# Gadersd/stable-diffusion-burn

Hardware: AMD Instinct MI355X
Metric: images/sec @512x512, 20-step DDIM CFG=7.5, SD v1.4 (higher is better)
Workload: dtype f32

## Files before the change

### ffi/sdmi.rs

```rust
use std::error::Error;
use std::ffi::{c_char, c_double, c_float, c_int, c_void, CStr, CString};

#[repr(C)]
pub struct SdmiConfig {
    pub device: i32,
    pub model_channels: i32,
    pub n_head: i32,
    pub ctx_dim: i32,
    pub latent_h: i32,
    pub latent_w: i32,
    pub vae_ch: i32,
    pub max_batch: i32,
    pub precision: i32,
    pub clip_layers: i32,
    pub clip_heads: i32,
    pub clip_vocab: i32,
    pub clip_ctx: i32,
    pub unet_in_ch: i32,
    pub reserved: [i32; 2],
}

impl SdmiConfig {
    pub fn control_hint_ch(&self) -> i32 { self.reserved[0] }
    pub fn set_control_hint_ch(&mut self, v: i32) { self.reserved[0] = v; }
    pub fn variant(&self) -> i32 { self.reserved[1] }
    pub fn set_variant(&mut self, v: i32) { self.reserved[1] = v; }
}

#[repr(C)]
#[derive(Default, Debug, Clone, Copy)]
pub struct SdmiAttnPlan {
    pub kernel: i32,
    pub waves: i32,
    pub q_rows: i32,
    pub kv_tile: i32,
    pub kv_splits: i32,
    pub reserved: [i32; 3],
}

#[repr(C)]
pub struct SdmiControl {
    pub hint_rgb: *const u8,
    pub n_hint: i32,
    pub hint_h: i32,
    pub hint_w: i32,
    pub strength: f64,
    pub start: f64,
    pub end: f64,
    pub reserved: [i64; 4],
}

#[repr(C)]
pub struct SdmiSampler {
    pub kind: i32,
    pub reserved0: i32,
    pub eta: f64,
    pub noise_seed: u64,
    pub image_base: i64,
    pub reserved: [i64; 4],
}
// ... 764 lines not shown
```

### include/sdmi.h

```cpp
#ifndef SDMI_H
#define SDMI_H

#include <stddef.h>
#include <stdint.h>

#ifdef __cplusplus
extern "C" {
#endif

typedef struct sdmi_ctx sdmi_ctx;

typedef enum sdmi_status {
    SDMI_OK = 0,
    SDMI_ERR_INVALID = -1,
    SDMI_ERR_HIP = -2,
    SDMI_ERR_WEIGHTS = -3,
    SDMI_ERR_IO = -4,
    SDMI_ERR_UNSUPPORTED = -5,
    SDMI_ERR_STATE = -6
} sdmi_status;

typedef struct sdmi_config {
    int32_t device;
    int32_t model_channels;
// ... 288 lines not shown
                   float* out);
int sdmi_op_unpack_tensor(sdmi_ctx* ctx, const void* raw, int32_t dtype, int32_t ndim, const int64_t* dims, int32_t transform, float* out);
int sdmi_op_geglu_forward(sdmi_ctx* ctx, const float* x, const float* weight, const float* bias, int32_t rows, int32_t cin,
                          int32_t hidden, float* out);
int sdmi_op_timestep_embedding(sdmi_ctx* ctx, int32_t t, int32_t dim, float* out);
int sdmi_op_timestep_embedding_f(sdmi_ctx* ctx, double t, int32_t dim, float* out);

int sdmi_set_option(sdmi_ctx* ctx, const char* key, const char* value);
int sdmi_last_call_stats(sdmi_ctx* ctx, double* gpu_ms, int64_t* n_kernels, double* flops);
int sdmi_profile_stats(sdmi_ctx* ctx, int32_t cls, double* ms, int64_t* launches, double* flops, double* bytes);
int sdmi_profile_overhead(sdmi_ctx* ctx, double* ms);
int sdmi_bench_conv(sdmi_ctx* ctx, int32_t n, int32_t cin, int32_t h, int32_t w, int32_t cout,
                    int32_t k, int32_t stride, int32_t upsample2x, int32_t tile_cfg, int32_t splitk,
                    int32_t iters, double* ms_out);

int sdmi_bench_attention(sdmi_ctx* ctx, int32_t n, int32_t nq, int32_t nk, int32_t n_state, int32_t n_head,
                         int32_t iters, double* ms_out);
typedef struct sdmi_attn_plan {
    int32_t kernel;
    int32_t waves;
    int32_t q_rows;
    int32_t kv_tile;
    int32_t kv_splits;
    int32_t reserved[3];
} sdmi_attn_plan;
int sdmi_attention_plan(sdmi_ctx* ctx, int32_t n, int32_t n_head, int32_t nq, int32_t nk, int32_t d_head, int32_t has_mask, sdmi_attn_plan* out);

#ifdef __cplusplus
}
#endif
#endif
```

### stable_diffusion_burn_amd/_capi.py

```python
from __future__ import annotations

import ctypes as C
import os
import sys
from pathlib import Path

_PKG = Path(__file__).resolve().parent
LIB_PATH = _PKG / "lib" / "libsdmi.so"


class SdmiError(RuntimeError):
    def __init__(self, status: int, message: str):
        super().__init__(f"sdmi status {status}: {message}")
        self.status = status


class SdmiConfig(C.Structure):
    _fields_ = [
        ("device", C.c_int32), ("model_channels", C.c_int32), ("n_head", C.c_int32), ("ctx_dim", C.c_int32),
        ("latent_h", C.c_int32), ("latent_w", C.c_int32), ("vae_ch", C.c_int32), ("max_batch", C.c_int32),
        ("precision", C.c_int32), ("clip_layers", C.c_int32), ("clip_heads", C.c_int32), ("clip_vocab", C.c_int32),
        ("clip_ctx", C.c_int32), ("unet_in_ch", C.c_int32), ("reserved", C.c_int32 * 2),
    ]

    @property
    def control_hint_ch(self) -> int:
        return int(self.reserved[0])

    @control_hint_ch.setter
    def control_hint_ch(self, v: int) -> None:
        self.reserved[0] = int(v)

    @property
    def variant(self) -> int:
        return int(self.reserved[1])

    @variant.setter
    def variant(self, v: int) -> None:
        self.reserved[1] = int(v)


class SdmiAttnPlan(C.Structure):
    _fields_ = [("kernel", C.c_int32), ("waves", C.c_int32), ("q_rows", C.c_int32), ("kv_tile", C.c_int32), ("kv_splits", C.c_int32), ("reserved", C.c_int32 * 3)]


class SdmiOpView(C.Structure):
    _fields_ = [("in_ld", C.c_int32), ("in_off", C.c_int32), ("out_ld", C.c_int32), ("out_off", C.c_int32), ("in_fill", C.c_float),
                ("in_planes", C.c_int32), ("out_planes", C.c_int32)]


class SdmiSampler(C.Structure):
    _fields_ = [("kind", C.c_int32), ("reserved0", C.c_int32), ("eta", C.c_double), ("noise_seed", C.c_uint64), ("image_base", C.c_int64),
                ("reserved", C.c_int64 * 4)]


class SdmiKSampler(C.Structure):
    _fields_ = [("kind", C.c_int32), ("schedule", C.c_int32), ("eta", C.c_double), ("rho", C.c_double), ("sigma_min", C.c_double), ("sigma_max", C.c_double),
                ("noise_seed", C.c_uint64), ("image_base", C.c_int64), ("reserved", C.c_int64 * 4)]


class SdmiControl(C.Structure):
    _fields_ = [("hint_rgb", C.POINTER(C.c_uint8)), ("n_hint", C.c_int32), ("hint_h", C.c_int32), ("hint_w", C.c_int32), ("strength", C.c_double),
                ("start", C.c_double), ("end", C.c_double), ("reserved", C.c_int64 * 4)]


class SdmiInpaint(C.Structure):
# ... 188 lines not shown
```

### stable_diffusion_burn_amd/csrc/attn_plan.cpp

```cpp
#include "attn_plan.hpp"

#include <algorithm>

#include "error.hpp"

namespace sdmi {

static const int kCUs = 256;

static long long workgroups(const AttnPlanIn& p, int rows) { return (long long)((p.nq + rows - 1) / rows) * p.n * p.n_head; }

static AttnPlan form(const AttnPlanIn& p, AttnKernel k, int waves, int kv_splits = 1, int wpe = 1, int qr = 1) {
    const AttnGeom& g = *attn_geom(k, p.d_head, qr);
    AttnPlan a{};
    a.kernel = k; a.waves = waves; a.wpe = wpe; a.qr = qr;
    a.q_rows = g.rows_per_wave * waves; a.kv_tile = g.kv_tile; a.kv_splits = kv_splits;
    return a;
}

static int plan_kv_splits(const AttnPlanIn& p, const AttnPlanOpts& o, bool on_split) {
    if (p.bf16 || p.has_mask || o.attn_kv_splits == 1) return 1;
    const AttnGeom& g = *attn_geom(on_split ? AttnKernel::Split : AttnKernel::Flash, p.d_head);
    const int tiles = (p.nk + g.kv_tile - 1) / g.kv_tile;
    if (o.attn_kv_splits > 1) return std::min(o.attn_kv_splits, std::max(1, tiles));
    const long long most = std::min(tiles / 2, 8);
    const long long wgs4 = workgroups(p, 4 * g.rows_per_wave);
    long long s = std::min<long long>(wgs4 > 0 && wgs4 <= kCUs / 2 ? kCUs / wgs4 : 1, most);
    if (on_split && o.attn_kv_prefer8) {
        const long long wgs8 = workgroups(p, 8 * g.rows_per_wave);
        const long long s8 = std::min<long long>(wgs8 < kCUs ? (kCUs + wgs8 - 1) / wgs8 : 1, most);
        if (s8 >= 2 && wgs8 * s8 >= kCUs) s = s8;
    }
    return (int)std::max<long long>(1, s);
}

static bool d64_stays_on_flash(const AttnPlanIn& p, const AttnPlanOpts& o) {
    if (p.nq <= 64) return false;
    const int tiles = (p.nk + 63) / 64;
    const int sf = plan_kv_splits(p, o, false), ss = plan_kv_splits(p, o, true);
    if (workgroups(p, 64) * sf > kCUs) return false;
    const int tf = (tiles + sf - 1) / sf, ts = (tiles + ss - 1) / ss;
    return 8 * tf + (sf > 1 ? 15 : 0) <= 9 * ts + (ss > 1 ? 15 : 0);
}

static AttnPlan plan_flash(const AttnPlanIn& p, int kv_splits) {
    return form(p, AttnKernel::Flash, 2 * workgroups(p, 128) >= 3 * kCUs ? 8 : 4, kv_splits);
}

static AttnPlan plan_split(const AttnPlanIn& p, const AttnPlanOpts& o, int kv_splits) {
    const bool pk = p.d_head == 40 && (o.attn_pack_tail & 1), lg = (o.attn_pack_tail & 2) != 0;
    const bool w8 = workgroups(p, 256) * kv_splits >= kCUs && (lg || p.d_head != 80);
    AttnPlan a = form(p, AttnKernel::Split, w8 ? 8 : 4, kv_splits);
    a.pk = pk; a.lg = lg;
    return a;
}

static AttnPlan plan_bf16(const AttnPlanIn& p, const AttnPlanOpts& o) {
    const int v = o.attn_bf16_variant, d = p.d_head;
    const bool force = (v & 0x100) != 0, short_ctx = p.nk <= 128;
    auto fills = [&](int rows, int per_cu) { return workgroups(p, rows) >= per_cu * kCUs; };
    if (d == 40) {
        if ((v & 4) && (force ? !(v & 2) : short_ctx && fills(256, 2))) return form(p, AttnKernel::Bf16, 4, 1, 2, 2);
        if ((v & 2) && (force || (!short_ctx && fills(512, 1)))) return form(p, AttnKernel::Bf16, 8, 1, 2, 2);
    }
    if ((d == 40 || d == 80) && (v & 1) && (force || (short_ctx && fills(128, 2)))) return form(p, AttnKernel::Bf16, 4, 1, 2);
    for (int waves : {8, 4})
        if (fills(32 * waves, 1)) return form(p, AttnKernel::Bf16, waves);
    return form(p, AttnKernel::Bf16, 2);
}

AttnPlan plan_attention(const AttnPlanIn& p, const AttnPlanOpts& o) {
    const int d = p.d_head;
    const bool fused = attn_supported_head_dim(d);
    if (p.planes_out && (p.bf16 || !fused || (p.n_head * d) % 32)) throw Error(SDMI_ERR_STATE, "attention: plane output needs a fused fp32 kernel");
    if (!fused) {
        if (p.has_mask) throw Error(SDMI_ERR_UNSUPPORTED, "attention: additive mask is only supported for head dims 40/80/160");
        if (d % 32) throw Error(SDMI_ERR_UNSUPPORTED, "attention: head dim must be 40/80/160 or a multiple of 32");
        if (p.bf16 && (d % 64)) throw Error(SDMI_ERR_UNSUPPORTED, "bf16 attention (unfused path): head dim must be a multiple of 64");
        AttnPlan a{};
        a.kernel = AttnKernel::Unfused; a.kv_splits = 1;
        return a;
    }
    if (p.bf16 && p.has_mask) throw Error(SDMI_ERR_UNSUPPORTED, "attention: additive mask is fp32-only");
    if (p.bf16 && o.attn_bf16 && attn_bf16_head_dim(d, o.attn_d64)) return plan_bf16(p, o);
    const bool on_split = !p.bf16 && !p.has_mask && o.attn_split && p.rows_aligned && attn_split_head_dim(d, o.attn_d64) && !(d == 64 && o.attn_d64 == 2 && d64_stays_on_flash(p, o));
    const int kv_splits = plan_kv_splits(p, o, on_split);
    return on_split ? plan_split(p, o, kv_splits) : plan_flash(p, kv_splits);
}

}
```

### stable_diffusion_burn_amd/csrc/attn_plan.hpp

```cpp
#pragma once

namespace sdmi {

enum class AttnKernel {
    Unfused,
    Flash,
    Split,
    Bf16,
};

struct AttnGeom { AttnKernel kernel; int d_head, qr, rows_per_wave, kv_tile; };
inline constexpr AttnGeom kAttnGeom[] = {
    {AttnKernel::Flash, 40, 1, 16, 64}, {AttnKernel::Flash, 64, 1, 16, 64}, {AttnKernel::Flash, 80, 1, 16, 64}, {AttnKernel::Flash, 160, 1, 16, 32},
    {AttnKernel::Split, 40, 1, 32, 64}, {AttnKernel::Split, 64, 1, 32, 64}, {AttnKernel::Split, 80, 1, 32, 64},
    {AttnKernel::Bf16, 40, 1, 32, 128}, {AttnKernel::Bf16, 40, 2, 64, 64},
    {AttnKernel::Bf16, 64, 1, 32, 64}, {AttnKernel::Bf16, 80, 1, 32, 64}, {AttnKernel::Bf16, 160, 1, 32, 64},
};
constexpr const AttnGeom* attn_geom(AttnKernel k, int d_head, int qr = 1) {
    for (const AttnGeom& g : kAttnGeom)
        if (g.kernel == k && g.d_head == d_head && g.qr == qr) return &g;
    return nullptr;
}
constexpr bool attn_supported_head_dim(int d) { return attn_geom(AttnKernel::Flash, d) != nullptr; }
constexpr bool attn_bf16_head_dim(int d, int attn_d64 = 0) { return attn_geom(AttnKernel::Bf16, d) != nullptr && (d != 64 || attn_d64); }
constexpr bool attn_split_head_dim(int d, int attn_d64 = 0) { return attn_geom(AttnKernel::Split, d) != nullptr && (d != 64 || attn_d64); }

struct AttnPlanIn {
    int n, n_head, nq;
    int nk;
    int d_head;
    int bf16;
    bool has_mask;
    bool planes_out;
    bool rows_aligned;
};

struct AttnPlanOpts {
    int attn_split = 1;
    int attn_bf16 = 1;
    int attn_bf16_variant = 7;
    int attn_pack_tail = 3;
    int attn_kv_splits = 0;
    int attn_kv_prefer8 = 1;
    int attn_d64 = 0;
};

struct AttnPlan {
    AttnKernel kernel;
    int waves;
    bool pk, lg;
    int wpe, qr;
    int q_rows;
    int kv_tile;
    int kv_splits;
};

AttnPlan plan_attention(const AttnPlanIn& in, const AttnPlanOpts& o);

}
```

### stable_diffusion_burn_amd/csrc/engine.cpp

```cpp
#include "engine.hpp"
#include "ckpt_keys.hpp"
#include "lora_keys.hpp"
#include "mpk_reader.hpp"
#include "safetensors_reader.hpp"

#include <dlfcn.h>

#include <algorithm>
#include <cmath>
#include <cstdarg>
#include <cstdio>
#include <cstring>
#include <fstream>
#include <sstream>

namespace sdmi {

static constexpr size_t kAlign = 256;
static constexpr size_t kSlabMin = (size_t)1 << 30;

DevPool::~DevPool() {
    for (auto& s : slabs_) (void)hipFree(s.base);
}

// ... 168 lines not shown
}
void Engine::roctx_push(const char* name) { if (g_roctx.push) (void)g_roctx.push(name); }
void Engine::roctx_pop() { if (g_roctx.pop) (void)g_roctx.pop(); }

Engine::Engine(const sdmi_config& cfg) : cfg_(cfg) {
    if (cfg.precision < 0 || cfg.precision > 2) throw Error(SDMI_ERR_UNSUPPORTED, "precision must be 0 (fp32), 1 (bf16) or 2 (bf16 + MXFP8 ResBlock convolutions)");
    bf16_ = cfg.precision >= 1;
    fp8_ = cfg.precision == 2;
    if (bf16_ && (cfg.model_channels % 64 || cfg.vae_ch % 64 || cfg.ctx_dim % 64))
        throw Error(SDMI_ERR_UNSUPPORTED, "precision=1 (bf16) needs model_channels, vae_ch and ctx_dim to be multiples of 64");
    if (cfg.model_channels % 32 || cfg.model_channels <= 0) throw Error(SDMI_ERR_INVALID, "model_channels must be a positive multiple of 32");
    if (cfg.vae_ch % 32 || cfg.vae_ch <= 0) throw Error(SDMI_ERR_INVALID, "vae_ch must be a positive multiple of 32");
    if (cfg.variant != 0 && cfg.variant != 1) throw Error(SDMI_ERR_INVALID, "variant must be 0 (SD v1) or 1 (SD 2.x)");
    if (cfg.variant == 1 && cfg.model_channels % 64) throw Error(SDMI_ERR_INVALID, "variant = 1 (SD 2.x): model_channels must be a multiple of 64, the head width");
    if (cfg.variant == 0 && (cfg.n_head <= 0 || cfg.model_channels % cfg.n_head)) throw Error(SDMI_ERR_INVALID, "n_head must divide model_channels");
    if (cfg.ctx_dim % 32 || cfg.ctx_dim <= 0) throw Error(SDMI_ERR_INVALID, "ctx_dim must be a positive multiple of 32");
    if (cfg_.unet_in_ch == 0) cfg_.unet_in_ch = 4;
    if (cfg_.unet_in_ch < 4 || cfg_.unet_in_ch > 12) throw Error(SDMI_ERR_INVALID, "unet_in_ch must be 4 (the latent alone) or 5 .. 12 (the latent + conditioning channels)");
    if (cfg_.control_hint_ch != 0 && cfg_.control_hint_ch != 3) throw Error(SDMI_ERR_INVALID, "control_hint_ch must be 0 (no ControlNet) or 3 (an RGB hint)");
    if (cfg_.control_hint_ch != 0 && cfg_.unet_in_ch != 4)
        throw Error(SDMI_ERR_UNSUPPORTED, "control_hint_ch != 0 needs unet_in_ch = 4: the control encoder's first convolution takes the 4 latent channels");
    if (cfg_.control_hint_ch != 0 && cfg_.variant == 1) throw Error(SDMI_ERR_UNSUPPORTED, "control_hint_ch != 0 is not supported on a variant = 1 (SD 2.x) context");
    aopt_.attn_d64 = cfg_.variant == 1 ? 2 : 0;
    check_latent_size(cfg.latent_h, cfg.latent_w);
    lat_h_ = cfg.latent_h;
    lat_w_ = cfg.latent_w;
    int ndev = 0;
    SDMI_HIP(hipGetDeviceCount(&ndev));
    if (ndev <= 0) throw Error(SDMI_ERR_HIP, "no HIP device visible: libsdmi has no CPU fallback");
    if (cfg.device < 0 || cfg.device >= ndev) throw Error(SDMI_ERR_INVALID, "device ordinal out of range");
    SDMI_HIP(hipSetDevice(cfg.device));
    hipDeviceProp_t prop;
    SDMI_HIP(hipGetDeviceProperties(&prop, cfg.device));
    if (std::string(prop.gcnArchName).find("gfx950") == std::string::npos)
        throw Error(SDMI_ERR_UNSUPPORTED, std::string("libsdmi is built for gfx950 (MI355X) only; device is ") + prop.gcnArchName);
    try {
    SDMI_HIP(hipStreamCreateWithFlags(&stream_, hipStreamNonBlocking));
    pool_.set_stream(stream_);
    SDMI_HIP(hipEventCreate(&ev0_));
    SDMI_HIP(hipEventCreate(&ev1_));
    SDMI_HIP(hipEventCreateWithFlags(&ev_user_, hipEventDisableTiming));
    SDMI_HIP(hipMalloc(&zero_page_, 256));
    weight_allocs_.push_back(zero_page_);
    SDMI_HIP(hipMemsetAsync(zero_page_, 0, 256, stream_));
    SDMI_HIP(hipStreamSynchronize(stream_));
    tuning_.load_builtin();
// ... 1292 lines not shown
    else if (key == "op_f32") opt_op_f32_ = std::stoi(value);
    else if (key == "pool_fill") {
        const int b = std::stoi(value);
        if (b < -1 || b > 255) throw Error(SDMI_ERR_INVALID, "pool_fill: -1 (off) or a byte 0 .. 255");
        pool_.set_fill(b);
        if (b >= 0 && std::none_of(entries_.begin(), entries_.end(), [](const WeightEntry& w) { return w.set; })) {
            SDMI_HIP(hipSetDevice(cfg_.device));
            for (const PersistentBlock& pb : persistent_blocks_) {
                SDMI_HIP(hipMemsetAsync(pb.p, b, pb.bytes, stream_));
                pool_.note_fill(pb.bytes);
            }
        }
    }
    else if (key == "dump_pool_fills") {
        std::ofstream f(value);
        if (!f) throw Error(SDMI_ERR_IO, "dump_pool_fills: cannot write " + value);
        unsigned long long blocks = 0, bytes = 0;
        pool_.take_fill_counts(&blocks, &bytes);
        f << blocks << " " << bytes << "\n";
    }
    else if (key == "cfg_share") opt_cfg_share_ = std::stoi(value);
    else if (key == "attn_kv_splits") aopt_.attn_kv_splits = std::stoi(value);
    else if (key == "attn_kv_prefer8") aopt_.attn_kv_prefer8 = std::stoi(value);
    else if (key == "b3_grouped") {
        if (!entries_.empty() && std::any_of(entries_.begin(), entries_.end(), [](const WeightEntry& w) { return w.set; }))
            throw Error(SDMI_ERR_STATE, "b3_grouped selects the layout the weight planes are packed in: set it before the first weight is loaded");
        opt_b3_grouped_ = std::stoi(value);
    }
    else if (key == "keep_masters") {
        if (std::any_of(entries_.begin(), entries_.end(), [](const WeightEntry& w) { return w.set; }) || arena_done_[0] || arena_done_[1] || arena_done_[2] || arena_done_[3])
            throw Error(SDMI_ERR_STATE, "keep_masters decides what the weight arenas hold: set it before the first weight is loaded");
        opt_keep_masters_ = std::stoi(value) != 0;
    }
    else if (key == "attn_pack_tail") aopt_.attn_pack_tail = (value == "default") ? AttnPlanOpts().attn_pack_tail : std::stoi(value);
    else if (key == "gn32_min_wgs") opt_gn32_min_wgs_ = (opt_gn32_min_wgs_ & ~0xFFFF) | (std::stoi(value) & 0xFFFF);
    else if (key == "gn32_stats_min_wgs") opt_gn32_min_wgs_ = (opt_gn32_min_wgs_ & 0xFFFF) | ((std::stoi(value) + 1) << 16);
    else if (key == "gn_target_wgs") gn_tune_.target_wgs = std::stoi(value);
    else if (key == "gn_max_threads") gn_tune_.max_threads = std::stoi(value);
    else if (key == "gn_unroll") gn_tune_.unroll = std::stoi(value);
    else if (key == "fp8_tile") opt_fp8_tile_ = (value == "auto") ? -1 : std::stoi(value);
    else if (key == "resid_acc") opt_resid_acc_ = std::stoi(value);
    else if (key == "attn_bf16") aopt_.attn_bf16 = std::stoi(value);
    else if (key == "attn_bf16_variant") aopt_.attn_bf16_variant = (value == "default") ? AttnPlanOpts().attn_bf16_variant : std::stoi(value, nullptr, 0);
    else if (key == "attn_split") aopt_.attn_split = std::stoi(value);
    else if (key == "attn_d64") {
        const int v = (value == "default") ? (cfg_.variant == 1 ? 2 : 0) : std::stoi(value);
// ... 459 lines not shown

void Engine::attention(const float* q, int ldq, long long q_bs, const float* k, int ldk, long long k_bs,
                       const float* v, int ldv, long long v_bs, float* o, int ldo, long long o_bs, int n, int nq,
                       int nk, int n_head, int d_head, const int* kv_len_dev, const int* kv_len_host,
                       const float* mask, int mask_ld, int dt, void* o3, bool q_log2) {
    if (dt < 0) dt = edt();
    if (nq <= 0 || nk <= 0) throw Error(SDMI_ERR_INVALID, "attention: empty sequence");
    AttnPlanIn in{};
    in.n = n; in.n_head = n_head; in.nq = nq; in.nk = nk; in.d_head = d_head; in.bf16 = dt; in.has_mask = mask != nullptr; in.planes_out = o3 != nullptr;
    in.rows_aligned = !((ldq | ldk | ldv | ldo) & (dt ? 7 : 3));
    const AttnPlan plan = plan_attention(in, aopt_);
    if (q_log2 != q_prescaled(dt, d_head)) throw Error(SDMI_ERR_STATE, "attention: the caller's statement about the query's scale does not match the storage type / head dim");
    const float scale = q_log2 ? 0.83255461115769775635f : (float)std::pow((double)d_head, -0.25);
    if (plan.kernel != AttnKernel::Unfused) {
        AttnParams p{};
        p.q = q; p.k = k; p.v = v; p.o = o; p.kv_len = kv_len_dev; p.mask = mask; p.mask_ld = mask_ld;
        p.n = n; p.n_head = n_head; p.nq = nq; p.nk = nk; p.d_head = d_head;
        p.ldq = ldq; p.ldk = ldk; p.ldv = ldv; p.ldo = ldo;
        p.q_bs = q_bs; p.k_bs = k_bs; p.v_bs = v_bs; p.o_bs = o_bs; p.scale = scale;
        p.bf16 = dt;
        p.q_log2 = q_log2 ? 1 : 0;
        p.o3 = o3; p.ldo3 = (n_head * d_head / 32) * 192;
        const double fl = 4.0 * n * n_head * (double)nq * nk * d_head;
        const int kv_splits = plan.kv_splits;
        std::unique_ptr<Buf> part_o, part_ml;
        if (kv_splits > 1) {
            part_o.reset(new Buf(this, (size_t)kv_splits * n * nq * n_head * d_head * sizeof(float)));
            part_ml.reset(new Buf(this, (size_t)kv_splits * n * n_head * nq * 2 * sizeof(float)));
            p.kv_splits = kv_splits; p.part_o = part_o->f(); p.part_ml = part_ml->f();
        }
        ProfScope ps(this, PC_ATTENTION, fl, 0, kv_splits > 1 ? 2 : 1);
        ps.set_tag("attention n%d nq%d nk%d h%d d%d slices=%d", n, nq, nk, n_head, d_head, kv_splits);
        if (plan.kernel == AttnKernel::Bf16) SDMI_HIP(launch_attention_bf16(p, plan, stream_));
        else if (plan.kernel == AttnKernel::Split) SDMI_HIP(launch_attention_split(p, plan, stream_));
        else SDMI_HIP(launch_attention(p, plan, stream_));
        count_kernel(fl);
        if (kv_splits > 1) {
            SDMI_HIP(launch_attention_combine(p, stream_));
            count_kernel();
        }
        return;
    }
    for (int b = 0; b < n; ++b)
        if ((kv_len_host ? kv_len_host[b] : nk) % (dt ? 64 : 32)) throw Error(SDMI_ERR_UNSUPPORTED, "attention (unfused path): key count must be a multiple of 32 (64 for bf16)");
    for (int b = 0; b < n; ++b) {
        const int nkb = kv_len_host ? kv_len_host[b] : nk;
        Buf s(this, (size_t)nq * nkb * sizeof(float));
        Buf pb(this, dt ? (size_t)nq * nkb * 2 : 256);
        Buf vt(this, (size_t)d_head * nkb * (dt ? 2 : 4));
        for (int h = 0; h < n_head; ++h) {
            const float* qb = adv(q, b * q_bs + h * d_head, dt);
            const float* kb = adv(k, b * k_bs + h * d_head, dt);
            const float* vb = adv(v, b * v_bs + h * d_head, dt);
            float* ob = adv(o, b * o_bs + h * d_head, dt);
            ConvGemm g{};
// ... 2065 lines not shown
```

### stable_diffusion_burn_amd/csrc/k_attn.hip

```cpp
#include "kernels.hpp"
#include "k_split3.hpp"

namespace sdmi {

typedef float f32x4 __attribute__((ext_vector_type(4)));
typedef float f32x2 __attribute__((ext_vector_type(2)));
typedef unsigned int u32x4h __attribute__((ext_vector_type(4)));
typedef unsigned int u32x2h __attribute__((ext_vector_type(2)));

__device__ __forceinline__ void swap32(float a, float b, float& ra, float& rb) {
    asm volatile("s_nop 1\n\tv_permlane32_swap_b32 %0, %1" : "+v"(a), "+v"(b));
    ra = a;
    rb = b;
}
__device__ __forceinline__ void swap16(float a, float b, float& ra, float& rb) {
    asm volatile("s_nop 1\n\tv_permlane16_swap_b32 %0, %1" : "+v"(a), "+v"(b));
    ra = a;
    rb = b;
}
__device__ __forceinline__ float xlane_max4(float v) {
    float a, b;
    swap32(v, v, a, b);
    v = fmaxf(a, b);
    swap16(v, v, a, b);
// ... 233 lines not shown
            return;
        }
    }
    const float inv = 1.0f / xlane_sum4(l_run);
    if (q_ok) {
#pragma unroll
        for (int dt = 0; dt < DT; ++dt) {
            const int dcol = dt * 16 + g * 4;
            if (dcol < D) {
                const f32x4 r = o[dt] * inv;
                if constexpr (H16) {
                    auto bits = [](float f) { unsigned u = __float_as_uint(f); u += 0x7FFFu + ((u >> 16) & 1u); return u >> 16; };
                    u32x2h w = {bits(r[0]) | (bits(r[1]) << 16), bits(r[2]) | (bits(r[3]) << 16)};
                    *reinterpret_cast<u32x2h*>(Oh + (long long)qrow * p.ldo + dcol) = w;
                } else {
                    if (p.o3) s3_store4(reinterpret_cast<unsigned char*>(p.o3) + ((long long)b * p.nq + qrow) * p.ldo3, hh * D + dcol, r);
                    else *reinterpret_cast<f32x4*>(Ob + (long long)qrow * p.ldo + dcol) = r;
                }
            }
        }
    }
}

__global__ __launch_bounds__(256) void softmax_rows_kernel(float* x, int rows, int cols, float scale) {
    __shared__ float red[8];
    const int row = blockIdx.x;
    if (row >= rows) return;
    float* xr = x + (long long)row * cols;
    const int tid = threadIdx.x, lane = tid & 63, wave = tid >> 6;
    float mx = -INFINITY;
    for (int i = tid; i < cols; i += 256) mx = fmaxf(mx, xr[i] * scale);
    for (int off = 32; off > 0; off >>= 1) mx = fmaxf(mx, __shfl_xor(mx, off));
    if (lane == 0) red[wave] = mx;
    __syncthreads();
    mx = fmaxf(fmaxf(red[0], red[1]), fmaxf(red[2], red[3]));
    float sum = 0.f;
    for (int i = tid; i < cols; i += 256) {
        const float e = __expf(xr[i] * scale - mx);
        xr[i] = e;
        sum += e;
    }
    for (int off = 32; off > 0; off >>= 1) sum += __shfl_xor(sum, off);
    if (lane == 0) red[4 + wave] = sum;
    __syncthreads();
    sum = (red[4] + red[5]) + (red[6] + red[7]);
    const float inv = 1.0f / sum;
// ... 65 lines not shown
            for (int s = 0; s < p.kv_splits; ++s) {
                const f32x2 ml = *reinterpret_cast<const f32x2*>(p.part_ml + ((((long long)s * p.n + b) * p.n_head + hh) * p.nq + q) * 2);
                if (ml[0] == -INFINITY) continue;
                const float w = __builtin_amdgcn_exp2f(ml[0] - m);
                acc += *reinterpret_cast<const f32x4*>(p.part_o + (((long long)s * p.n + b) * p.nq + q) * row_elems + hh * D + c4 * 4) * w;
                l += ml[1] * w;
            }
        }
        const f32x4 r = acc * (1.0f / l);
        if (p.o3) s3_store4(reinterpret_cast<unsigned char*>(p.o3) + ((long long)b * p.nq + q) * p.ldo3, hh * D + c4 * 4, r);
        else *reinterpret_cast<f32x4*>(p.o + (long long)b * p.o_bs + (long long)q * p.ldo + hh * D + c4 * 4) = r;
    }
}

hipError_t launch_attention_combine(const AttnParams& p, hipStream_t stream) {
    if (p.kv_splits < 2 || !p.part_o || !p.part_ml || p.bf16 || (p.d_head & 3) || (!p.o3 && (p.ldo & 3))) return hipErrorInvalidValue;
    const long long total = (long long)p.n * p.nq * p.n_head * (p.d_head >> 2);
    long long blocks = (total + 255) / 256;
    if (blocks > 4096) blocks = 4096;
    hipLaunchKernelGGL(attn_combine_kernel, dim3((unsigned)blocks), dim3(256), 0, stream, p);
    return hipGetLastError();
}

hipError_t launch_attention(const AttnParams& p, const AttnPlan& plan, hipStream_t stream) {
    if (plan.kernel != AttnKernel::Flash || plan.kv_splits != (p.kv_splits > 1 ? p.kv_splits : 1)) return hipErrorInvalidValue;
    if (p.kv_splits > 1 && (p.bf16 || p.mask || !p.part_o || !p.part_ml)) return hipErrorInvalidValue;
    switch (p.d_head) {
        case 40: return launch_attn2_any<40>(p, plan, stream);
        case 64: return launch_attn2_any<64>(p, plan, stream);
        case 80: return launch_attn2_any<80>(p, plan, stream);
        case 160: return launch_attn2_any<160>(p, plan, stream);
    }
    return hipErrorInvalidValue;
}

hipError_t launch_softmax_rows(float* x, int rows, int cols, float scale, hipStream_t stream) {
    hipLaunchKernelGGL(softmax_rows_kernel, dim3(rows), dim3(256), 0, stream, x, rows, cols, scale);
    return hipGetLastError();
}

}
```

### stable_diffusion_burn_amd/csrc/sdmi_capi.cpp

```cpp
#include <algorithm>
#include <climits>
#include <cmath>
#include <cstdint>
#include <cstdio>
#include <cstring>
#include <map>
#include <memory>
#include <string>
#include <vector>

#include "engine.hpp"
#include "ckpt_keys.hpp"
#include "mpk_reader.hpp"
#include "prompt.hpp"
#include "safetensors_reader.hpp"
#include "lora_keys.hpp"
#include "tokenizer.hpp"

using sdmi::Engine;
using sdmi::Error;

namespace sdmi {
void write_png_rgb8(const std::string& path, const uint8_t* rgb, int width, int height);
}
// ... 1679 lines not shown

int sdmi_bench_conv(sdmi_ctx* ctx, int32_t n, int32_t cin, int32_t h, int32_t w, int32_t cout, int32_t k,
                    int32_t stride, int32_t upsample2x, int32_t tile_cfg, int32_t splitk, int32_t iters, double* ms_out) {
    return guarded([&] {
        if (!ms_out) throw Error(SDMI_ERR_INVALID, "bench_conv: null output");
        *ms_out = eng(ctx).bench_conv(n, cin, h, w, cout, k, stride, upsample2x ? 1 : 0, tile_cfg, splitk, iters);
    });
}

int sdmi_bench_attention(sdmi_ctx* ctx, int32_t n, int32_t nq, int32_t nk, int32_t n_state, int32_t n_head,
                         int32_t iters, double* ms_out) {
    return guarded([&] {
        if (!ms_out) throw Error(SDMI_ERR_INVALID, "bench_attention: null output");
        *ms_out = eng(ctx).bench_attention(n, nq, nk, n_state, n_head, iters);
    });
}

int sdmi_attention_plan(sdmi_ctx* ctx, int32_t n, int32_t n_head, int32_t nq, int32_t nk, int32_t d_head, int32_t has_mask, sdmi_attn_plan* out) {
    return guarded([&] {
        if (!out) throw Error(SDMI_ERR_INVALID, "attention_plan: null output");
        const sdmi::AttnPlan a = eng(ctx).attention_plan(n, n_head, nq, nk, d_head, has_mask != 0);
        *out = sdmi_attn_plan{};
        out->kernel = a.kernel == sdmi::AttnKernel::Unfused ? 0 : a.kernel == sdmi::AttnKernel::Flash ? 1 : a.kernel == sdmi::AttnKernel::Split ? 2 : 3;
        out->waves = a.waves; out->q_rows = a.q_rows; out->kv_tile = a.kv_tile; out->kv_splits = a.kv_splits;
    });
}

}
```

### stable_diffusion_burn_amd/pipeline.py

```python
from __future__ import annotations

import ctypes as C
import os
import re
from dataclasses import dataclass

import numpy as np

from . import _capi
from ._capi import SdmiAttnPlan, SdmiConfig, SdmiControl, SdmiError, SdmiHires, SdmiInpaint, SdmiKSampler, SdmiOpView, SdmiPromptOpts, SdmiSampler, check, load_library

def mpk_list(path) -> list:
    lib = load_library()
    need = C.c_size_t()
    check(lib.sdmi_mpk_list(str(path).encode(), None, 0, C.byref(need)))
    buf = C.create_string_buffer(need.value)
    check(lib.sdmi_mpk_list(str(path).encode(), buf, need.value, C.byref(need)))
    out = []
    for line in buf.value.decode().splitlines():
        if line.startswith("#") or not line:
            continue
        name, shape, off = line.split("\t")
        out.append((name, tuple(int(v) for v in shape.split(",")) if shape else (), int(off)))
    return out
# ... 1004 lines not shown

    def profile_stats(self) -> dict:
        out = {}
        for i, name in enumerate(self.PROFILE_CLASSES):
            ms, n, fl, by = C.c_double(), C.c_int64(), C.c_double(), C.c_double()
            check(self._lib.sdmi_profile_stats(self._ctx, i, C.byref(ms), C.byref(n), C.byref(fl), C.byref(by)))
            out[name] = {"ms": ms.value, "launches": n.value, "flops": fl.value, "bytes": by.value}
        return out

    def bench_conv(self, n, cin, h, w, cout, k=3, stride=1, upsample2x=0, tile_cfg=-1, splitk=0, iters=10) -> float:
        ms = C.c_double()
        check(self._lib.sdmi_bench_conv(self._ctx, n, cin, h, w, cout, k, stride, upsample2x, tile_cfg, splitk, iters,
                                        C.byref(ms)))
        return ms.value

    def set_prediction(self, kind: str = "eps") -> None:
        check(self._lib.sdmi_set_prediction(self._ctx, _prediction(kind)))

    ATTN_KERNELS = ("unfused", "flash", "split", "bf16")

    def attention_plan(self, n, n_head, nq, nk, d_head, has_mask=False) -> dict:
        p = SdmiAttnPlan()
        check(self._lib.sdmi_attention_plan(self._ctx, int(n), int(n_head), int(nq), int(nk), int(d_head), int(bool(has_mask)), C.byref(p)))
        return {"kernel": self.ATTN_KERNELS[p.kernel], "waves": int(p.waves), "q_rows": int(p.q_rows), "kv_tile": int(p.kv_tile), "kv_splits": int(p.kv_splits)}

    def bench_attention(self, n, nq, nk, n_state, n_head, iters=10) -> float:
        ms = C.c_double()
        check(self._lib.sdmi_bench_attention(self._ctx, n, nq, nk, n_state, n_head, iters, C.byref(ms)))
        return ms.value

    def op_unpack_tensor(self, raw, dtype: str, transform: int = 0) -> np.ndarray:
        code = {"F32": 0, "F16": 1, "BF16": 2}[dtype]
        raw = np.ascontiguousarray(raw, dtype={0: np.float32, 1: np.float16, 2: np.uint16}[code])
        shape = raw.shape
        if transform == 1:
            out_shape = shape[::-1]
        elif transform == 2:
            out_shape = (shape[0], (shape[1] + 3) // 4 * 4) + tuple(shape[2:])
        else:
            out_shape = shape
        out = np.empty(out_shape, np.float32)
        dims = (C.c_int64 * raw.ndim)(*shape)
        check(self._lib.sdmi_op_unpack_tensor(self._ctx, raw.ctypes.data_as(C.c_void_p), code, raw.ndim, dims, int(transform), _fp(out)))
        return out

    def op_resize(self, x, out_size, mode="bicubic", antialias: bool = False):
        x = _f32(x)
# ... 558 lines not shown
```

Before: 4.361.

## Add intra-workgroup KV-sliced flash attention for head dim 160

Adds a flash-attention kernel in which several wave groups inside one workgroup each process a slice of the KV tiles, then merge their partial softmax results through LDS. This replaces the cross-workgroup kv-split path, with its global partial buffers and separate merge, for short-KV cases such as the d_head=160 attention layers. The planner enables it automatically for fp32 when KV tiles are few and the workgroup count is at most the CU count. The cost is much more LDS per workgroup, which may lower occupancy, plus a new code path to maintain.

```diff
diff --git a/ffi/sdmi.rs b/ffi/sdmi.rs
--- a/ffi/sdmi.rs
+++ b/ffi/sdmi.rs
@@ -35,7 +35,8 @@
     pub q_rows: i32,
     pub kv_tile: i32,
     pub kv_splits: i32,
-    pub reserved: [i32; 3],
+    pub wg_slices: i32,
+    pub reserved: [i32; 2],
 }
 
 #[repr(C)]
diff --git a/include/sdmi.h b/include/sdmi.h
--- a/include/sdmi.h
+++ b/include/sdmi.h
@@ -334,7 +334,8 @@
     int32_t q_rows;
     int32_t kv_tile;
     int32_t kv_splits;
-    int32_t reserved[3];
+    int32_t wg_slices;
+    int32_t reserved[2];
 } sdmi_attn_plan;
 int sdmi_attention_plan(sdmi_ctx* ctx, int32_t n, int32_t n_head, int32_t nq, int32_t nk, int32_t d_head, int32_t has_mask, sdmi_attn_plan* out);
 
diff --git a/stable_diffusion_burn_amd/_capi.py b/stable_diffusion_burn_amd/_capi.py
--- a/stable_diffusion_burn_amd/_capi.py
+++ b/stable_diffusion_burn_amd/_capi.py
@@ -41,7 +41,7 @@
 
 
 class SdmiAttnPlan(C.Structure):
-    _fields_ = [("kernel", C.c_int32), ("waves", C.c_int32), ("q_rows", C.c_int32), ("kv_tile", C.c_int32), ("kv_splits", C.c_int32), ("reserved", C.c_int32 * 3)]
+    _fields_ = [("kernel", C.c_int32), ("waves", C.c_int32), ("q_rows", C.c_int32), ("kv_tile", C.c_int32), ("kv_splits", C.c_int32), ("wg_slices", C.c_int32), ("reserved", C.c_int32 * 2)]
 
 
 class SdmiOpView(C.Structure):
diff --git a/stable_diffusion_burn_amd/csrc/attn_plan.cpp b/stable_diffusion_burn_amd/csrc/attn_plan.cpp
--- a/stable_diffusion_burn_amd/csrc/attn_plan.cpp
+++ b/stable_diffusion_burn_amd/csrc/attn_plan.cpp
@@ -14,7 +14,7 @@
     const AttnGeom& g = *attn_geom(k, p.d_head, qr);
     AttnPlan a{};
     a.kernel = k; a.waves = waves; a.wpe = wpe; a.qr = qr;
-    a.q_rows = g.rows_per_wave * waves; a.kv_tile = g.kv_tile; a.kv_splits = kv_splits;
+    a.q_rows = g.rows_per_wave * waves; a.kv_tile = g.kv_tile; a.kv_splits = kv_splits; a.wg_slices = 1;
     return a;
 }
 
@@ -41,6 +41,23 @@
     if (workgroups(p, 64) * sf > kCUs) return false;
     const int tf = (tiles + sf - 1) / sf, ts = (tiles + ss - 1) / ss;
     return 8 * tf + (sf > 1 ? 15 : 0) <= 9 * ts + (ss > 1 ? 15 : 0);
+}
+
+static const int kWgMaxWorkgroups = kCUs;
+static const int kWgMaxTilesPerSlice = 2;
+static int plan_wg_slices(const AttnPlanIn& p, const AttnPlanOpts& o, bool on_split) {
+    if (o.attn_wg_slices <= 0 || p.bf16 || p.has_mask) return 1;
+    const AttnKernel k = on_split ? AttnKernel::Split : AttnKernel::Flash;
+    const AttnWgGeom* w = attn_wg_geom(k, p.d_head);
+    if (!w) return 1;
+    const AttnGeom& g = *attn_geom(k, p.d_head);
+    const int tiles = (p.nk + g.kv_tile - 1) / g.kv_tile;
+    if (o.attn_wg_slices > 1) return o.attn_wg_slices <= tiles && o.attn_wg_slices <= w->max_slices ? o.attn_wg_slices : 1;
+    if (o.attn_kv_splits != 0) return 1;
+    if (tiles < 2 || workgroups(p, g.rows_per_wave * w->row_waves) > kWgMaxWorkgroups) return 1;
+    const int s = std::min(tiles, w->max_slices);
+    if ((tiles + s - 1) / s > kWgMaxTilesPerSlice) return 1;
+    return s;
 }
 
 static AttnPlan plan_flash(const AttnPlanIn& p, int kv_splits) {
@@ -78,12 +95,20 @@
         if (d % 32) throw Error(SDMI_ERR_UNSUPPORTED, "attention: head dim must be 40/80/160 or a multiple of 32");
         if (p.bf16 && (d % 64)) throw Error(SDMI_ERR_UNSUPPORTED, "bf16 attention (unfused path): head dim must be a multiple of 64");
         AttnPlan a{};
-        a.kernel = AttnKernel::Unfused; a.kv_splits = 1;
+        a.kernel = AttnKernel::Unfused; a.kv_splits = 1; a.wg_slices = 1;
         return a;
     }
     if (p.bf16 && p.has_mask) throw Error(SDMI_ERR_UNSUPPORTED, "attention: additive mask is fp32-only");
     if (p.bf16 && o.attn_bf16 && attn_bf16_head_dim(d, o.attn_d64)) return plan_bf16(p, o);
     const bool on_split = !p.bf16 && !p.has_mask && o.attn_split && p.rows_aligned && attn_split_head_dim(d, o.attn_d64) && !(d == 64 && o.attn_d64 == 2 && d64_stays_on_flash(p, o));
+    if (const int s = plan_wg_slices(p, o, on_split); s > 1) {
+        const AttnKernel k = on_split ? AttnKernel::Split : AttnKernel::Flash;
+        const int rw = attn_wg_geom(k, d)->row_waves;
+        AttnPlan a = form(p, k, rw * s, s);
+        a.q_rows = attn_geom(k, d)->rows_per_wave * rw;
+        a.wg_slices = s;
+        return a;
+    }
     const int kv_splits = plan_kv_splits(p, o, on_split);
     return on_split ? plan_split(p, o, kv_splits) : plan_flash(p, kv_splits);
 }
diff --git a/stable_diffusion_burn_amd/csrc/attn_plan.hpp b/stable_diffusion_burn_amd/csrc/attn_plan.hpp
--- a/stable_diffusion_burn_amd/csrc/attn_plan.hpp
+++ b/stable_diffusion_burn_amd/csrc/attn_plan.hpp
@@ -25,6 +25,17 @@
 constexpr bool attn_bf16_head_dim(int d, int attn_d64 = 0) { return attn_geom(AttnKernel::Bf16, d) != nullptr && (d != 64 || attn_d64); }
 constexpr bool attn_split_head_dim(int d, int attn_d64 = 0) { return attn_geom(AttnKernel::Split, d) != nullptr && (d != 64 || attn_d64); }
 
+inline constexpr int kLdsBytesPerCU = 160 * 1024;
+struct AttnWgGeom { AttnKernel kernel; int d_head, row_waves, max_slices; };
+inline constexpr AttnWgGeom kAttnWgGeom[] = {
+    {AttnKernel::Flash, 160, 1, 3},
+};
+constexpr const AttnWgGeom* attn_wg_geom(AttnKernel k, int d_head) {
+    for (const AttnWgGeom& g : kAttnWgGeom)
+        if (g.kernel == k && g.d_head == d_head) return &g;
+    return nullptr;
+}
+
 struct AttnPlanIn {
     int n, n_head, nq;
     int nk;
@@ -43,6 +54,7 @@
     int attn_kv_splits = 0;
     int attn_kv_prefer8 = 1;
     int attn_d64 = 0;
+    int attn_wg_slices = 0;
 };
 
 struct AttnPlan {
@@ -53,6 +65,7 @@
     int q_rows;
     int kv_tile;
     int kv_splits;
+    int wg_slices;
 };
 
 AttnPlan plan_attention(const AttnPlanIn& in, const AttnPlanOpts& o);
diff --git a/stable_diffusion_burn_amd/csrc/engine.cpp b/stable_diffusion_burn_amd/csrc/engine.cpp
--- a/stable_diffusion_burn_amd/csrc/engine.cpp
+++ b/stable_diffusion_burn_amd/csrc/engine.cpp
@@ -214,6 +214,7 @@
         throw Error(SDMI_ERR_UNSUPPORTED, "control_hint_ch != 0 needs unet_in_ch = 4: the control encoder's first convolution takes the 4 latent channels");
     if (cfg_.control_hint_ch != 0 && cfg_.variant == 1) throw Error(SDMI_ERR_UNSUPPORTED, "control_hint_ch != 0 is not supported on a variant = 1 (SD 2.x) context");
     aopt_.attn_d64 = cfg_.variant == 1 ? 2 : 0;
+    aopt_.attn_wg_slices = bf16_ ? 0 : 1;
     check_latent_size(cfg.latent_h, cfg.latent_w);
     lat_h_ = cfg.latent_h;
     lat_w_ = cfg.latent_w;
@@ -1552,6 +1553,11 @@
     else if (key == "cfg_share") opt_cfg_share_ = std::stoi(value);
     else if (key == "attn_kv_splits") aopt_.attn_kv_splits = std::stoi(value);
     else if (key == "attn_kv_prefer8") aopt_.attn_kv_prefer8 = std::stoi(value);
+    else if (key == "attn_wg_slices") {
+        const int v = (value == "default") ? (bf16_ ? 0 : 1) : std::stoi(value);
+        if (v < 0) throw Error(SDMI_ERR_INVALID, "attn_wg_slices: 0 (never), 1 (automatic) or the slice count to force");
+        aopt_.attn_wg_slices = v;
+    }
     else if (key == "b3_grouped") {
         if (!entries_.empty() && std::any_of(entries_.begin(), entries_.end(), [](const WeightEntry& w) { return w.set; }))
             throw Error(SDMI_ERR_STATE, "b3_grouped selects the layout the weight planes are packed in: set it before the first weight is loaded");
@@ -2057,7 +2063,7 @@
         p.q_log2 = q_log2 ? 1 : 0;
         p.o3 = o3; p.ldo3 = (n_head * d_head / 32) * 192;
         const double fl = 4.0 * n * n_head * (double)nq * nk * d_head;
-        const int kv_splits = plan.kv_splits;
+        const int kv_splits = plan.wg_slices > 1 ? 1 : plan.kv_splits;
         std::unique_ptr<Buf> part_o, part_ml;
         if (kv_splits > 1) {
             part_o.reset(new Buf(this, (size_t)kv_splits * n * nq * n_head * d_head * sizeof(float)));
@@ -2065,7 +2071,7 @@
             p.kv_splits = kv_splits; p.part_o = part_o->f(); p.part_ml = part_ml->f();
         }
         ProfScope ps(this, PC_ATTENTION, fl, 0, kv_splits > 1 ? 2 : 1);
-        ps.set_tag("attention n%d nq%d nk%d h%d d%d slices=%d", n, nq, nk, n_head, d_head, kv_splits);
+        ps.set_tag("attention n%d nq%d nk%d h%d d%d slices=%d%s", n, nq, nk, n_head, d_head, plan.kv_splits, plan.wg_slices > 1 ? " wg" : "");
         if (plan.kernel == AttnKernel::Bf16) SDMI_HIP(launch_attention_bf16(p, plan, stream_));
         else if (plan.kernel == AttnKernel::Split) SDMI_HIP(launch_attention_split(p, plan, stream_));
         else SDMI_HIP(launch_attention(p, plan, stream_));
diff --git a/stable_diffusion_burn_amd/csrc/k_attn.hip b/stable_diffusion_burn_amd/csrc/k_attn.hip
--- a/stable_diffusion_burn_amd/csrc/k_attn.hip
+++ b/stable_diffusion_burn_amd/csrc/k_attn.hip
@@ -279,6 +279,225 @@
     }
 }
 
+template <int D, int RW, int S>
+struct Attn2WgCfg {
+    using G = Attn2Cfg<D, RW, false>;
+    static constexpr int NT = RW * S * 64;
+    static constexpr int GROUP_FLOATS = 2 * G::TILE_FLOATS;
+    static constexpr int MERGE_FLOATS = RW * (G::DT * 256 + 128);
+    static constexpr size_t LDS_BYTES = (size_t)S * GROUP_FLOATS * sizeof(float);
+    static_assert(MERGE_FLOATS <= GROUP_FLOATS, "a group's partial result must fit its own K / V region");
+};
+
+template <int D, int RW, int S>
+__global__ __launch_bounds__(RW * S * 64) void attn2_wg_kernel(const AttnParams p) {
+    using Cfg = Attn2Cfg<D, RW, false>;
+    using Wg = Attn2WgCfg<D, RW, S>;
+    constexpr int NT = Cfg::NT, BKV = Cfg::BKV, KT = Cfg::KT, DT = Cfg::DT, DC = Cfg::DC, LDK = Cfg::LDK, NLD = Cfg::NLD;
+    constexpr float kLog2e = 1.4426950408889634f;
+
+    extern __shared__ __attribute__((aligned(16))) float smem[];
+
+    const int lane = threadIdx.x & 63;
+    const int wave = threadIdx.x >> 6;
+    const int grp = wave / RW;
+    const int rw = wave - grp * RW;
+    const int tid = rw * 64 + lane;
+    const int g = lane >> 4;
+    const int c = lane & 15;
+    float* Ks = smem + grp * Wg::GROUP_FLOATS;
+    float* Vs = Ks + Cfg::TILE_FLOATS;
+
+    const int b = blockIdx.y / p.n_head;
+    const int hh = blockIdx.y - b * p.n_head;
+    const int qrow = blockIdx.x * (16 * RW) + rw * 16 + c;
+    const bool q_ok = qrow < p.nq;
+
+    const float* Qb = p.q + (long long)b * p.q_bs + hh * D;
+    const float* Kb = p.k + (long long)b * p.k_bs + hh * D;
+    const float* Vb = p.v + (long long)b * p.v_bs + hh * D;
+    float* Ob = p.o + (long long)b * p.o_bs + hh * D;
+
+    const int nk = p.kv_len ? p.kv_len[b] : p.nk;
+    const int n_tiles = (nk + BKV - 1) / BKV;
+    const int n_full = nk / BKV;
+    const int tps = (n_tiles + S - 1) / S;
+    const int t_begin = min(grp * tps, n_tiles), t_end = min(t_begin + tps, n_tiles);
+
+    f32x4 rk[NLD], rv[NLD];
+    auto gload = [&](int tile) {
+        const int kv0 = tile * BKV;
+#pragma unroll
+        for (int i = 0; i < NLD; ++i) {
+            const int idx = tid + i * NT;
+            const int row = idx / (D / 4);
+            const int c4 = idx - row * (D / 4);
+            const int key = kv0 + row;
+            f32x4 kk = {0.f, 0.f, 0.f, 0.f}, vv = {0.f, 0.f, 0.f, 0.f};
+            if (idx < Cfg::F4_PER_TILE && key < nk) {
+                kk = *reinterpret_cast<const f32x4*>(Kb + (long long)key * p.ldk + c4 * 4);
+                vv = *reinterpret_cast<const f32x4*>(Vb + (long long)key * p.ldv + c4 * 4);
+            }
+            rk[i] = kk;
+            rv[i] = vv;
+        }
+    };
+    auto lstore = [&]() {
+#pragma unroll
+        for (int i = 0; i < NLD; ++i) {
+            const int idx = tid + i * NT;
+            if (idx < Cfg::F4_PER_TILE) {
+                const int row = idx / (D / 4);
+                const int c4 = idx - row * (D / 4);
+                const bool sw = (row & 8) != 0;
+                *reinterpret_cast<f32x4*>(Ks + row * LDK + c4 * 4) = sw ? f32x4{rk[i][2], rk[i][3], rk[i][0], rk[i][1]} : rk[i];
+                *reinterpret_cast<f32x4*>(Vs + row * LDK + c4 * 4) = rv[i];
+            }
+        }
+    };
+
+    f32x4 o[DT];
+#pragma unroll
+    for (int dt = 0; dt < DT; ++dt) o[dt] = f32x4{0.f, 0.f, 0.f, 0.f};
+    float m_run = -INFINITY;
+    float l_run = 0.f;
+
+    if (t_begin < t_end) gload(t_begin);
+    const float qscale = p.scale * p.scale * kLog2e;
+    f32x2 qf[DC];
+#pragma unroll
+    for (int cc = 0; cc < DC; ++cc) {
+        f32x2 v = {0.f, 0.f};
+        if (q_ok) v = *reinterpret_cast<const f32x2*>(Qb + (long long)qrow * p.ldq + cc * 8 + g * 2);
+        qf[cc] = v * qscale;
+    }
+    if (t_begin < t_end) lstore();
+    __syncthreads();
+
+    for (int it = 0; it < tps; ++it) {
+        const int tile = t_begin + it;
+        const bool live = tile < t_end;
+        const bool more = (tile + 1) < t_end;
+        if (more) gload(tile + 1);
+
+        if (live) {
+            const int kv0 = tile * BKV;
+            f32x4 s[KT];
+#pragma unroll
+            for (int kt = 0; kt < KT; ++kt) {
+                f32x4 a = {0.f, 0.f, 0.f, 0.f};
+                const float* kp = Ks + (kt * 16 + c) * LDK + ((g * 2) ^ ((c >> 3) << 1));
+#pragma unroll
+                for (int cc = 0; cc < DC; ++cc) {
+                    const f32x2 kf = *reinterpret_cast<const f32x2*>(kp + cc * 8);
+                    a = __builtin_amdgcn_mfma_f32_16x16x4f32(kf[0], qf[cc][0], a, 0, 0, 0);
+                    a = __builtin_amdgcn_mfma_f32_16x16x4f32(kf[1], qf[cc][1], a, 0, 0, 0);
+                }
+                s[kt] = a;
+            }
+
+            if (tile >= n_full) {
+#pragma unroll
+                for (int kt = 0; kt < KT; ++kt) {
+#pragma unroll
+                    for (int r = 0; r < 4; ++r) {
+                        const int key = kv0 + kt * 16 + g * 4 + r;
+                        float v = s[kt][r];
+                        if (key >= nk) v = -INFINITY;
+                        s[kt][r] = v;
+                    }
+                }
+            }
+
+            float mt = s[0][0];
+#pragma unroll
+            for (int kt = 0; kt < KT; ++kt)
+#pragma unroll
+                for (int r = 0; r < 4; ++r) mt = fmaxf(mt, s[kt][r]);
+            mt = xlane_max4(mt);
+            const float m_new = fmaxf(m_run, mt);
+            const float m_use = (m_new == -INFINITY) ? 0.f : m_new;
+            const float alpha = __builtin_amdgcn_exp2f(m_run - m_use);
+            float psum = 0.f;
+#pragma unroll
+            for (int kt = 0; kt < KT; ++kt) {
+#pragma unroll
+                for (int r = 0; r < 4; ++r) {
+                    const float e = __builtin_amdgcn_exp2f(s[kt][r] - m_use);
+                    s[kt][r] = e;
+                    psum += e;
+                }
+            }
+            l_run = l_run * alpha + psum;
+            m_run = m_new;
+#pragma unroll
+            for (int dt = 0; dt < DT; ++dt) o[dt] *= alpha;
+
+#pragma unroll
+            for (int kt = 0; kt < KT; ++kt) {
+#pragma unroll
+                for (int r = 0; r < 4; ++r) {
+                    const float* vp = Vs + (kt * 16 + g * 4 + r) * LDK + c;
+                    const float pv = s[kt][r];
+#pragma unroll
+                    for (int dt = 0; dt < DT; ++dt) o[dt] = __builtin_amdgcn_mfma_f32_16x16x4f32(vp[dt * 16], pv, o[dt], 0, 0, 0);
+                }
+            }
+        }
+
+        if (it + 1 < tps) {
+            __syncthreads();
+            if (more) lstore();
+            __syncthreads();
+        }
+    }
+
+    const float l_tot = xlane_sum4(l_run);
+    float* mo = Ks + rw * (DT * 256 + 128);
+    if constexpr (RW > 1) __syncthreads();
+    if (grp > 0) {
+#pragma unroll
+        for (int dt = 0; dt < DT; ++dt) *reinterpret_cast<f32x4*>(mo + (dt * 64 + lane) * 4) = o[dt];
+        *reinterpret_cast<f32x2*>(mo + DT * 256 + lane * 2) = f32x2{m_run, l_tot};
+    }
+    __syncthreads();
+    if (grp > 0) return;
+
+    f32x2 ml[S];
+    ml[0] = f32x2{m_run, l_tot};
+#pragma unroll
+    for (int s = 1; s < S; ++s) ml[s] = *reinterpret_cast<const f32x2*>(mo + s * Wg::GROUP_FLOATS + DT * 256 + lane * 2);
+    float m = -INFINITY;
+#pragma unroll
+    for (int s = 0; s < S; ++s) m = fmaxf(m, ml[s][0]);
+    float w[S];
+    float l = 0.f;
+#pragma unroll
+    for (int s = 0; s < S; ++s) {
+        w[s] = 0.f;
+        if (ml[s][0] != -INFINITY) {
+            w[s] = __builtin_amdgcn_exp2f(ml[s][0] - m);
+            l += ml[s][1] * w[s];
+        }
+    }
+    const float inv = 1.0f / l;
+#pragma unroll
+    for (int dt = 0; dt < DT; ++dt) {
+        f32x4 acc = {0.f, 0.f, 0.f, 0.f};
+#pragma unroll
+        for (int s = 0; s < S; ++s) {
+            const f32x4 po = s == 0 ? o[dt] : *reinterpret_cast<const f32x4*>(mo + s * Wg::GROUP_FLOATS + (dt * 64 + lane) * 4);
+            if (ml[s][0] != -INFINITY) acc += po * w[s];
+        }
+        const int dcol = dt * 16 + g * 4;
+        if (q_ok && dcol < D) {
+            const f32x4 r = acc * inv;
+            if (p.o3) s3_store4(reinterpret_cast<unsigned char*>(p.o3) + ((long long)b * p.nq + qrow) * p.ldo3, hh * D + dcol, r);
+            else *reinterpret_cast<f32x4*>(Ob + (long long)qrow * p.ldo + dcol) = r;
+        }
+    }
+}
+
 __global__ __launch_bounds__(256) void softmax_rows_kernel(float* x, int rows, int cols, float scale) {
     __shared__ float red[8];
     const int row = blockIdx.x;
@@ -390,7 +609,31 @@
     return hipGetLastError();
 }
 
+template <int D, int S>
+static hipError_t launch_attn2_wg(const AttnParams& p, const AttnPlan& plan, hipStream_t stream) {
+    constexpr const AttnWgGeom* wg = attn_wg_geom(AttnKernel::Flash, D);
+    static_assert(wg != nullptr && S >= 2 && S <= wg->max_slices, "attn_plan.hpp's kAttnWgGeom has no such form");
+    constexpr int RW = wg->row_waves;
+    using Cfg = Attn2WgCfg<D, RW, S>;
+    static_assert(Cfg::G::BKV == attn_geom(AttnKernel::Flash, D)->kv_tile, "attn_plan.hpp's table and Attn2Cfg disagree");
+    static_assert(attn_geom(AttnKernel::Flash, D)->rows_per_wave == 16, "attn_plan.hpp's table and attn2_wg_kernel's row mapping (qrow) disagree");
+    static_assert(Attn2WgCfg<D, RW, wg->max_slices>::LDS_BYTES <= (size_t)kLdsBytesPerCU && Attn2WgCfg<D, RW, wg->max_slices + 1>::LDS_BYTES > (size_t)kLdsBytesPerCU,
+                  "kAttnWgGeom's max_slices is not what fits the LDS");
+    if (plan.q_rows != 16 * RW || plan.waves != RW * S) return hipErrorInvalidValue;
+    auto k = attn2_wg_kernel<D, RW, S>;
+    if (hipError_t e = set_max_dynamic_lds(reinterpret_cast<const void*>(k), (int)Cfg::LDS_BYTES); e != hipSuccess) return e;
+    dim3 grid((p.nq + plan.q_rows - 1) / plan.q_rows, p.n * p.n_head, 1);
+    hipLaunchKernelGGL(k, grid, dim3(Cfg::NT), Cfg::LDS_BYTES, stream, p);
+    return hipGetLastError();
+}
+
 hipError_t launch_attention(const AttnParams& p, const AttnPlan& plan, hipStream_t stream) {
+    if (plan.kernel == AttnKernel::Flash && plan.wg_slices > 1) {
+        if (plan.kv_splits != plan.wg_slices || p.kv_splits > 1 || p.bf16 || p.mask) return hipErrorInvalidValue;
+        if (p.d_head == 160 && plan.wg_slices == 2) return launch_attn2_wg<160, 2>(p, plan, stream);
+        if (p.d_head == 160 && plan.wg_slices == 3) return launch_attn2_wg<160, 3>(p, plan, stream);
+        return hipErrorInvalidValue;
+    }
     if (plan.kernel != AttnKernel::Flash || plan.kv_splits != (p.kv_splits > 1 ? p.kv_splits : 1)) return hipErrorInvalidValue;
     if (p.kv_splits > 1 && (p.bf16 || p.mask || !p.part_o || !p.part_ml)) return hipErrorInvalidValue;
     switch (p.d_head) {
diff --git a/stable_diffusion_burn_amd/csrc/sdmi_capi.cpp b/stable_diffusion_burn_amd/csrc/sdmi_capi.cpp
--- a/stable_diffusion_burn_amd/csrc/sdmi_capi.cpp
+++ b/stable_diffusion_burn_amd/csrc/sdmi_capi.cpp
@@ -1725,8 +1725,8 @@
         const sdmi::AttnPlan a = eng(ctx).attention_plan(n, n_head, nq, nk, d_head, has_mask != 0);
         *out = sdmi_attn_plan{};
         out->kernel = a.kernel == sdmi::AttnKernel::Unfused ? 0 : a.kernel == sdmi::AttnKernel::Flash ? 1 : a.kernel == sdmi::AttnKernel::Split ? 2 : 3;
-        out->waves = a.waves; out->q_rows = a.q_rows; out->kv_tile = a.kv_tile; out->kv_splits = a.kv_splits;
-    });
-}
-
-}
+        out->waves = a.waves; out->q_rows = a.q_rows; out->kv_tile = a.kv_tile; out->kv_splits = a.kv_splits; out->wg_slices = a.wg_slices;
+    });
+}
+
+}
diff --git a/stable_diffusion_burn_amd/pipeline.py b/stable_diffusion_burn_amd/pipeline.py
--- a/stable_diffusion_burn_amd/pipeline.py
+++ b/stable_diffusion_burn_amd/pipeline.py
@@ -1050,7 +1050,8 @@
     def attention_plan(self, n, n_head, nq, nk, d_head, has_mask=False) -> dict:
         p = SdmiAttnPlan()
         check(self._lib.sdmi_attention_plan(self._ctx, int(n), int(n_head), int(nq), int(nk), int(d_head), int(bool(has_mask)), C.byref(p)))
-        return {"kernel": self.ATTN_KERNELS[p.kernel], "waves": int(p.waves), "q_rows": int(p.q_rows), "kv_tile": int(p.kv_tile), "kv_splits": int(p.kv_splits)}
+        return {"kernel": self.ATTN_KERNELS[p.kernel], "waves": int(p.waves), "q_rows": int(p.q_rows), "kv_tile": int(p.kv_tile), "kv_splits": int(p.kv_splits),
+                "wg_slices": int(p.wg_slices)}
 
     def bench_attention(self, n, nq, nk, n_state, n_head, iters=10) -> float:
         ms = C.c_double()
```

After: 4.357. No clear change (-0.1%).
